# bacpop/ska.rust

Measured on AMD Instinct MI355X. Metric: genomes/sec ska build+align, 1 000x5 Mbp k=31; bit-exact vs CPU, higher is better.
Workload: dtype u64

## Files before the change

ska.rust_amd/csrc/skx_api.cpp:

```cpp
#include "skx_internal.h"
#include "../../include/skx_host.h"
#include <algorithm>
#include <atomic>
#include <chrono>
#include <cmath>
#include <cstdarg>
#include <cstddef>
#include <cstdio>
#include <cstring>
#include <map>
#include <memory>
#include <mutex>
#include <numeric>
#include <optional>
#include <unordered_map>
#include <thread>
#include <cerrno>
#include <fcntl.h>
#include <sys/mman.h>
#include <sys/stat.h>
#include <unistd.h>

using namespace skx;

// ... 1057 lines not shown
    int missing = 0;
    SKX_HIP(hipMemcpyAsync(&missing, d_flag.p, 4, hipMemcpyDeviceToHost, st));
    SKX_HIP(hipStreamSynchronize(st));
    SKX_HIP(hipGetLastError());
    if (missing) { set_error("row keyset does not contain every split k-mer of the samples"); return SKX_EINVAL; }
    *out = a.release();
    return SKX_OK;
    });
}

static PiecesRowsArgs pieces_args(skx_array *a)
{
    PiecesRowsArgs pa{};
    const skx_pieces *pc = a->pieces; const skx_keyset *rows = a->lazy_rows;
    pa.pieces = pc->data.p; pa.plen = pc->plen.p; pa.perm = pc->perm.p; pa.nrank = pc->nrank.p; pa.cap = pc->cap; pa.n_samples = (int)a->names.size();
    pa.ncnt = rows->ncnt.p; pa.roff = rows->roff.p;
    return pa;
}
static void launch_assemble_lazy(skx_array *a, const AssembleArgs &aa, hipStream_t st, int mode, uint32_t n_blocks = 0)
{
    if (a->lazy_rows->wide) launch_assemble_wide(aa, st, mode, n_blocks); else launch_assemble(aa, st, mode, n_blocks);
}
static AssembleArgs lazy_args(skx_array *a, int *d_flag)
{
    AssembleArgs aa{};
    skx_keyset *rows = a->lazy_rows;
    aa.d = a->lazy_dict->view(); aa.logN = rows->logN; aa.stage = rows->stage.p; aa.stride = rows->stride; aa.ncnt = rows->ncnt.p; aa.roff = rows->roff.p;
    aa.matrix = nullptr; aa.pitch = 0; aa.col_present = a->present.p; aa.col_unambig = a->unambig.p; aa.col_mask = a->mask.p;
    aa.max_rows = rows->max_rows; aa.missing = d_flag;
    return aa;
// ... 184 lines not shown
        if (logQ > bits || attempt > 3) return not_taken("row blocks kept overflowing (a sample that is one repeat, or far more rows than the probe saw)");
        const uint64_t nsub = 1ull << logQ;
        const double mean = u_est / (double)nsub;
        const uint32_t cap = ranks_for(mean), nslots = slots_for(cap);
        const uint64_t amp = 1ull << (logQ - logB);
        const uint64_t amp_max = region_cap > (wide ? LDS_SORT_MAX_WIDE : LDS_SORT_MAX) ? 32 : 8;
        if (amp > amp_max && (double)raw_sum * (double)amp > 4e8) return not_taken("too many row blocks per region: every region would be read too often");
        if (!pass_ok(logQ, nslots, cap)) return not_taken("no row-block split that fits the LDS");
        std::unique_ptr<skx_keyset> ks(new skx_keyset());
        ks->ctx = ctx; ks->k = d->k; ks->rc = d->rc; ks->logN = logQ; ks->hp = d->hp; ks->wh = d->wh; ks->wide = wide; ks->stride = cap;
        std::unique_ptr<skx_pieces> pc(new skx_pieces());
        pc->cap = cap; pc->logQ = logQ;
        SKX_TRY(ks->stage.alloc(nsub * cap * wpk)); SKX_TRY(ks->ncnt.alloc(nsub));
        if (pc->data.alloc(nsub * (uint64_t)S * (cap / 2)) != SKX_OK) return not_taken("no room for the pieces");
        SKX_TRY(pc->plen.alloc(nsub * (uint64_t)S + 2)); SKX_TRY(pc->perm.alloc(nsub * cap)); SKX_TRY(pc->nrank.alloc(nsub));
        SKX_TRY(d_flag.zero(st));
        aa.logQ = logQ; aa.nslots = nslots; aa.cap = cap;
        aa.rounds = 1; aa.bar = nullptr;
        DevBuf<int> d_bar;
        {
            int cus = 0; (void)hipDeviceGetAttribute(&cus, hipDeviceAttributeMultiprocessorCount, ctx->device);
            uint64_t g = nsub;
            while (g > (uint64_t)std::max(cus, 1) && g % 2 == 0) g /= 2;
            if (g <= (uint64_t)std::max(cus, 1) && nsub % g == 0 && g % (8 * amp) == 0 && logB >= 3) {
                aa.rounds = (uint32_t)(nsub / g);
                SKX_TRY(d_bar.alloc(2ull << logB)); SKX_TRY(d_bar.zero(st)); aa.bar = d_bar.p;
            }
        }
        aa.pieces = pc->data.p; aa.plen = pc->plen.p; aa.perm = pc->perm.p; aa.nrank = pc->nrank.p;
        aa.stage = ks->stage.p; aa.stride = cap; aa.ncnt = ks->ncnt.p;
        { KernelTimer kt(ctx, &ctx->tm.append); if (wide) launch_append_wide(aa, st); else launch_append(aa, region_cap, st); }
        int ov = 0;
        SKX_HIP(hipMemcpyAsync(&ov, d_flag.p, 4, hipMemcpyDeviceToHost, st));
        SKX_HIP(hipStreamSynchronize(st));
        SKX_HIP(hipGetLastError());
        if (getenv("SKX_DEBUG")) fprintf(stderr, "[skx] append%s: logQ=%d (x%llu per region) cap=%u slots=%u rows~%.0f -> %s\n", wide ? " (128-bit keys)" : "", logQ, (unsigned long long)amp, cap, nslots, u_est, ov ? "overflow" : "ok");
        if (ov & 4) return not_taken("the table's bytes are not at LDS address 0");
        if (ov) continue;
        SKX_TRY(keyset_finish(ks.get()));
        ctx->merge_path = wide ? "append128" : "append64";
        ks_out = std::move(ks); pc_out = std::move(pc);
        return SKX_OK;
    }
}
// ... 23 lines not shown
        SKX_HIP(hipMemcpyAsync(blk->roff.p, ks->roff.p, (nsub + 1) * 8, hipMemcpyDeviceToDevice, st));
        blk->total = U; blk->max_rows = ks->max_rows;
    }
    std::unique_ptr<skx_array> a(new skx_array());
    a->ctx = ctx; a->k = d->k; a->rc = d->rc; a->k_bits = d->key_bits; a->hp = d->hp; a->wh = d->wh; a->version = skx_version();
    for (int i = 0; i < S; i++) a->names.emplace_back(names && names[i] ? names[i] : "");
    a->n_rows = a->n_kmers = U; a->pitch = 0; a->engine_order = true; a->stats_ready = true;
    SKX_TRY(a->present.alloc(U)); SKX_TRY(a->unambig.alloc(U)); SKX_TRY(a->mask.alloc(U)); SKX_TRY(a->keys.alloc(U * (d->wide() ? 2 : 1))); SKX_TRY(a->vcount.alloc(U));
    if (U) {
        skx_keyset *src = g ? g : ks;
        if (src->wide) launch_gather_keys_wide((const u128 *)src->stage.p, src->stride, g ? g->ncnt.p : blk->ncnt.p, g ? g->roff.p : blk->roff.p, 1 << src->logN, (u128 *)a->keys.p, st);
        else launch_gather_keys(src->stage.p, src->stride, g ? g->ncnt.p : blk->ncnt.p, g ? g->roff.p : blk->roff.p, 1 << src->logN, a->keys.p, 0, src->hp, st);
        if (g) { SKX_TRY(a->present.zero(st)); SKX_TRY(a->unambig.zero(st)); SKX_TRY(a->mask.zero(st)); SKX_TRY(a->vcount.zero(st)); }
        StageTimer t(ctx, &ctx->tm.assemble);
        KernelTimer kt(ctx, &ctx->tm.pieces_stats);
        launch_pieces_stats(pc->data.p, pc->plen.p, pc->perm.p, pc->nrank.p, blk->ncnt.p, blk->roff.p, pc->cap, S, 1 << logQ, a->present.p, a->unambig.p, a->mask.p, a->vcount.p, st);
    }
    SKX_HIP(hipStreamSynchronize(st));
    SKX_HIP(hipGetLastError());
    a->pieces = pc.release(); a->lazy_rows = blk.release();
    *out = a.release();
    return SKX_OK;
}
static int merge_append(skx_ctx *ctx, skx_dictset *d, const char *const *names, skx_array **out)
{
    std::unique_ptr<skx_keyset> ks; std::unique_ptr<skx_pieces> pc;
    const int r = append_pass(ctx, d, ks, pc);
    if (r != SKX_OK) return r;
    return array_over_pieces(ctx, d, ks.get(), pc.release(), nullptr, names, out);
}

// ... 250 lines not shown
    if (counts) for (uint64_t i = 0; i < U; i++) counts[i] = pres[idx[i]];
    return SKX_OK;
    });
}

extern "C" int skx_array_sample_kmers(skx_array *a, int64_t *out)
{
    return skx_guarded([&]() -> int {
    skx_ctx *ctx = a->ctx; hipStream_t st = ctx->stream;
    SKX_HIP(hipSetDevice(ctx->device));
    const size_t S = a->names.size();
    if (a->pieces) {
        skx_pieces *pc = a->pieces;
        if (pc->sample_cells.size() != S) {
            DevBuf<unsigned long long> d; SKX_TRY(d.alloc(S)); SKX_TRY(d.zero(st));
            launch_pieces_cells(pc->data.p, pc->plen.p, pc->cap, (int)S, 1 << pc->logQ, d.p, st);
            std::vector<unsigned long long> h(S);
            SKX_HIP(hipMemcpyAsync(h.data(), d.p, S * 8, hipMemcpyDeviceToHost, st));
            SKX_HIP(hipStreamSynchronize(st));
            pc->sample_cells.assign(h.begin(), h.end());
        }
        for (size_t i = 0; i < S; i++) out[i] = (int64_t)pc->sample_cells[i];
        return SKX_OK;
    }
    if (a->lazy()) { for (size_t i = 0; i < S; i++) out[i] = (int64_t)a->lazy_dict->sample_size[i]; return SKX_OK; }
    DevBuf<unsigned long long> d; SKX_TRY(d.alloc(S)); SKX_TRY(d.zero(st));
    launch_row_nonmissing(a->matrix.p, a->pitch, (int)S, a->n_rows, d.p, st);
    std::vector<unsigned long long> h(S);
    SKX_HIP(hipMemcpyAsync(h.data(), d.p, S * 8, hipMemcpyDeviceToHost, st));
    SKX_HIP(hipStreamSynchronize(st));
    for (size_t i = 0; i < S; i++) out[i] = (int64_t)h[i];
// ... 1 lines not shown
    });
}

extern "C" int skx_array_pieces_info(skx_array *a, uint64_t *piece_bytes, uint64_t *row_blocks, uint32_t *ranks_per_block)
{
    return skx_guarded([&]() -> int {
    if (!a) { set_error("bad arguments"); return SKX_EINVAL; }
    if (piece_bytes) *piece_bytes = 0;
    if (row_blocks) *row_blocks = 0;
    if (ranks_per_block) *ranks_per_block = 0;
    const skx_pieces *pc = a->pieces;
    if (!pc) return SKX_OK;
    skx_ctx *ctx = a->ctx; hipStream_t st = ctx->stream;
    SKX_HIP(hipSetDevice(ctx->device));
    const uint64_t n = ((uint64_t)1 << pc->logQ) * a->names.size();
    std::vector<uint16_t> h(n);
    SKX_HIP(hipMemcpyAsync(h.data(), pc->plen.p, n * 2, hipMemcpyDeviceToHost, st));
    SKX_HIP(hipStreamSynchronize(st));
    uint64_t b = 0;
    for (uint16_t v : h) b += ((uint64_t)v + 31) / 32 * 16;
    if (piece_bytes) *piece_bytes = b;
    if (row_blocks) *row_blocks = (uint64_t)1 << pc->logQ;
    if (ranks_per_block) *ranks_per_block = pc->cap;
    return SKX_OK;
    });
}

static int array_compact(skx_array *a, DevBuf<uint8_t> &keep, DevBuf<uint64_t> &pos, uint64_t kept, int mask_ambig, bool vcount_from_unambig,
                         bool keys_follow)
{
    skx_ctx *ctx = a->ctx; hipStream_t st = ctx->stream;
    const uint64_t U = a->n_rows; const size_t S = a->names.size();
    const bool filter_ambig_as_missing = vcount_from_unambig;
    if (kept == U && !mask_ambig) {
        if (filter_ambig_as_missing && U) SKX_HIP(hipMemcpyAsync(a->vcount.p, a->unambig.p, U * 4, hipMemcpyDeviceToDevice, st));
// ... 990 lines not shown
```

ska.rust_amd/csrc/skx_append.hip:

```cpp
#include "skx_device.h"
#include <cstdlib>
#include <type_traits>

namespace skx {

typedef uint32_t u32x4 __attribute__((ext_vector_type(4)));
typedef const u32x4 __attribute__((address_space(1))) *g4_t;

#ifdef SKX_AP_PROF
__device__ unsigned long long g_ap_prof[16];
#define AP_PROF_START unsigned long long tprof = __builtin_readcyclecounter(), tacc[12] = {0, 0, 0, 0, 0, 0, 0, 0, 0, 0, 0, 0}
#define AP_PROF(i) do { const unsigned long long t_ = __builtin_readcyclecounter(); tacc[(i)] += t_ - tprof; tprof = t_; } while (0)
#define AP_PROF_FLUSH() do { for (int i_ = 0; i_ < 12; i_++) if (tacc[i_] && (i_ >= 6 || (threadIdx.x & 63) == 0)) atomicAdd(&g_ap_prof[i_], tacc[i_]); } while (0)
extern "C" void skx_debug_phase_prof(unsigned long long *out, int reset)
{
    unsigned long long h[16];
    (void)hipDeviceSynchronize();
    (void)hipMemcpyFromSymbol(h, HIP_SYMBOL(g_ap_prof), sizeof(h));
    for (int i = 0; i < 16; i++) out[i] = h[i];
    if (reset) { for (auto &x : h) x = 0; (void)hipMemcpyToSymbol(HIP_SYMBOL(g_ap_prof), h, sizeof(h)); }
}
#else
#define AP_PROF_START do { } while (0)
#define AP_PROF(i) do { } while (0)
// ... 347 lines not shown
#endif
                }
#endif
            }
            if (last_chunk) {
                while (qw != qbase) { batch(std::false_type{}); AP_PROF(2); while (nsq >= 64u) { slow_batch(); AP_PROF(3); } }
                while (nsq) { slow_batch(); AP_PROF(3); }
            }
            AP_PROF(1);
            if (last_chunk) {
                if (!COUNT_ONLY) {
                    uint32_t n = *lds_vol(&s_ctl[CTL_NROWS]);
                    n = __builtin_amdgcn_readfirstlane(n);
                    if (n > cap) n = cap;
                    uint8_t *dst = piece0 + (uint64_t)s * (cap / 2);
                    for (uint32_t v = lane; v * 32u < n; v += 64u) {
                        uint4 *src = reinterpret_cast<uint4 *>(rb) + v;
                        const uint4 x = *src;
                        *reinterpret_cast<uint4 *>(dst + v * 16u) = x;
                        *src = make_uint4(0u, 0u, 0u, 0u);
                    }
                    if (lane == 0) a.plen[j * (uint64_t)S + s] = (uint16_t)n;
                }
                AP_PROF(4);
                if (!more) break;
                s += AP_WAVES; c = 0; off_c = off_n; cnt_c = cnt_n;
                if (AP_RESYNC > 0) {
                    const int it = (s - wv) / AP_WAVES;
                    if (xmap && A > 1u && a.bar && it % (AP_RESYNC > 0 ? AP_RESYNC : 1) == 0 && it <= (S - AP_WAVES) / AP_WAVES) {
                        __syncthreads();
                        if (tid == 0) {
                            int *ctr = a.bar + (1 << a.logB) + region;
                            const int want = (int)A * (it / (AP_RESYNC > 0 ? AP_RESYNC : 1));
                            atomicAdd(ctr, 1);
                            for (int spin = 0; spin < (1 << 16) && __hip_atomic_load(ctr, __ATOMIC_RELAXED, __HIP_MEMORY_SCOPE_AGENT) < want; spin++) __builtin_amdgcn_s_sleep(4);
// ... 62 lines not shown
    } else {
        (void)hipFuncSetAttribute((const void *)append_kernel<COUNT_ONLY, false>, hipFuncAttributeMaxDynamicSharedMemorySize, (int)lds);
        hipLaunchKernelGGL((append_kernel<COUNT_ONLY, false>), dim3(blocks), dim3(AP_THREADS), lds, st, a);
    }
}
bool append_ok(int bits, int logB, int logQ, uint32_t region_cap, uint32_t nslots, uint32_t cap)
{
    const int rem = bits - logQ;
    (void)region_cap;
    return logQ >= logB && rem >= 0 && rem <= 50 && cap % 128u == 0 && cap >= 128u && cap <= APPEND_MAX_CAP && nslots >= cap && (nslots & (nslots - 1u)) == 0u &&
           append_lds_bytes(nslots, cap, false) <= 160u * 1024u - 256u;
}
void launch_append(const AppendArgs &a, uint32_t region_cap, hipStream_t st) { (void)region_cap; launch_append_t<false>(a, (1u << a.logQ) / a.rounds, st); }
void launch_append_probe(const AppendArgs &a, uint32_t region_cap, unsigned blocks, hipStream_t st) { (void)region_cap; launch_append_t<true>(a, blocks, st); }

__global__ __launch_bounds__(256) void pieces_stats_kernel(const uint8_t *pieces, const uint16_t *plen, const uint16_t *perm, const uint32_t *nrank, const uint32_t *ncnt,
                                                           const uint64_t *roff, uint32_t cap, int S, uint32_t *o_present, uint32_t *o_unambig, uint32_t *o_mask,
                                                           uint32_t *o_vcount, int force_direct, uint32_t stage)
{
    constexpr int W = 4;
    extern __shared__ __attribute__((aligned(16))) uint16_t s_stage[];
    const uint32_t PS_STAGE = stage;
    uint16_t *const s_pr = s_stage, *const s_un = s_stage + stage, *const s_mk = s_stage + 2 * (size_t)stage;
    const uint64_t j = blockIdx.x;
    const uint32_t nr = nrank[j], nrows = ncnt[j];
    const uint64_t r0 = roff[j];
    const uint32_t d = blockIdx.y * 256u + threadIdx.x;
    if (blockIdx.y * 256u * 8u * W >= nr && !(blockIdx.y == 0 && nrows)) return;
    const bool staged = gridDim.y == 1 && nrows <= PS_STAGE && !force_direct;
    if (staged) {
        for (uint32_t p = threadIdx.x; p < nrows; p += 256) { s_pr[p] = 0; s_un[p] = 0; s_mk[p] = 0; }
        __syncthreads();
    }
    const int lane = threadIdx.x & 63, wv = threadIdx.x >> 6;
    const uint16_t *pl = plen + j * (uint64_t)S;
    const uint4 *col = reinterpret_cast<const uint4 *>(pieces + j * (uint64_t)S * (cap / 2)) + d;
    const uint32_t step = cap / 32;
    const bool mine = d * 32u < nr;
    uint32_t pN[W], aN[W];
    uint32_t pE[W], pO[W], aE[W], aO[W], uni[W];
    uint32_t PE0[W], PE1[W], PO0[W], PO1[W], AE0[W], AE1[W], AO0[W], AO1[W];
#pragma unroll
    for (int w = 0; w < W; w++) { pN[w] = aN[w] = 0; pE[w] = pO[w] = aE[w] = aO[w] = uni[w] = 0; PE0[w] = PE1[w] = PO0[w] = PO1[w] = AE0[w] = AE1[w] = AO0[w] = AO1[w] = 0; }
    auto nibfold = [&]() {
#pragma unroll
        for (int w = 0; w < W; w++) {
            pE[w] += pN[w] & 0x0F0F0F0Fu; pO[w] += (pN[w] >> 4) & 0x0F0F0F0Fu; aE[w] += aN[w] & 0x0F0F0F0Fu; aO[w] += (aN[w] >> 4) & 0x0F0F0F0Fu;
            pN[w] = aN[w] = 0;
        }
    };
// ... 5 lines not shown
            AE0[w] += aE[w] & 0x00FF00FFu; AE1[w] += (aE[w] >> 8) & 0x00FF00FFu; AO0[w] += aO[w] & 0x00FF00FFu; AO1[w] += (aO[w] >> 8) & 0x00FF00FFu;
            pE[w] = pO[w] = aE[w] = aO[w] = 0;
        }
    };
    auto take = [&](int w, uint32_t x) {
        uint32_t t = x | (x >> 1); t |= t >> 2;
        const uint32_t nz = t & 0x11111111u;
        const uint32_t y = x & (x - nz);
        uint32_t u = y | (y >> 1); u |= u >> 2;
        const uint32_t am = u & 0x11111111u;
        pN[w] += nz; aN[w] += am;
        uni[w] |= x;
    };
    for (int s0 = 0, since = 0, nib = 0; s0 < S; s0 += 64) {
        const uint32_t plv = s0 + lane < S ? (uint32_t)pl[s0 + lane] : 0u;
        const int n = S - s0 < 64 ? S - s0 : 64;
#pragma unroll 1
        for (int i0 = 0; i0 < n; i0 += 4) {
            if (nib == 12) { nibfold(); nib = 0; }
            nib += 4;
            uint4 x[4];
#pragma unroll
            for (int u = 0; u < 4; u++) {
                const uint32_t l = (uint32_t)__builtin_amdgcn_readlane((int)plv, (i0 + u) & 63);
                x[u] = make_uint4(0u, 0u, 0u, 0u);
                if (mine && i0 + u < n && d * 32u < l) x[u] = col[(uint64_t)(s0 + i0 + u) * step];
            }
#pragma unroll
            for (int u = 0; u < 4; u++) { take(0, x[u].x); take(1, x[u].y); take(2, x[u].z); take(3, x[u].w); }
        }
        since += 64;
        if (since >= 192) { fold(); since = 0; nib = 0; }
    }
    fold();
    const uint16_t *pj = perm + j * (uint64_t)cap;
    if (mine) {
#pragma unroll
        for (int w = 0; w < W; w++) {
            uint32_t pres[8], amb[8];
            pres[0] = PE0[w] & 0xFFFFu; pres[4] = PE0[w] >> 16; pres[2] = PE1[w] & 0xFFFFu; pres[6] = PE1[w] >> 16;
            pres[1] = PO0[w] & 0xFFFFu; pres[5] = PO0[w] >> 16; pres[3] = PO1[w] & 0xFFFFu; pres[7] = PO1[w] >> 16;
// ... 27 lines not shown
        uint32_t pp = 0xFFFFu; bool hit = false;
        if (rr < rk1) {
            pp = pj[rr];
            if (pp < nrows) {
                if (staged) hit = s_un[pp] != s_pr[pp];
                else hit = __hip_atomic_load(&o_unambig[r0 + pp], __ATOMIC_RELAXED, __HIP_MEMORY_SCOPE_AGENT) != __hip_atomic_load(&o_present[r0 + pp], __ATOMIC_RELAXED, __HIP_MEMORY_SCOPE_AGENT);
            }
        }
        unsigned long long todo = __ballot(hit);
        while (todo) {
            const int src = __builtin_ctzll(todo);
            todo &= todo - 1;
            const uint32_t r = rb + (uint32_t)src, prow = (uint32_t)__shfl((int)pp, src, 64);
            uint32_t m = 0;
            for (int t = lane; t < S; t += 64) {
                if ((uint32_t)pl[t] <= r) continue;
                const uint32_t x = *(reinterpret_cast<const uint32_t *>(pieces + (j * (uint64_t)S + t) * (cap / 2)) + (r >> 3));
                const uint32_t nib = (x >> ((r & 7u) * 4u)) & 15u;
                if (nib) m |= 1u << nib;
            }
#pragma unroll
            for (int dd = 32; dd >= 1; dd >>= 1) m |= __shfl_xor(m, dd, 64);
            if (lane == 0) { if (staged) s_mk[prow] = (uint16_t)m; else o_mask[r0 + prow] = m; }
        }
    }
    if (!staged) return;
    __syncthreads();
    for (uint32_t p = threadIdx.x; p < nrows; p += 256) {
        const uint32_t pr = s_pr[p];
        o_present[r0 + p] = pr; o_vcount[r0 + p] = pr;
        o_unambig[r0 + p] = s_un[p]; o_mask[r0 + p] = s_mk[p];
    }
}
void launch_pieces_stats(const uint8_t *pieces, const uint16_t *plen, const uint16_t *perm, const uint32_t *nrank, const uint32_t *ncnt, const uint64_t *roff, uint32_t cap,
                         int n_samples, int n_blocks, uint32_t *present, uint32_t *unambig, uint32_t *mask, uint32_t *vcount, hipStream_t st)
{
    if (n_blocks <= 0) return;
    const unsigned gy = (cap / 32 + 255u) / 256u;
    static const int direct = knob("stats_direct") ? 1 : 0;
    const uint32_t stage = (cap + 63u) / 64u * 64u;
    hipLaunchKernelGGL(pieces_stats_kernel, dim3((unsigned)n_blocks, gy), dim3(256), (size_t)stage * 6, st, pieces, plen, perm, nrank, ncnt, roff, cap, n_samples, present, unambig, mask, vcount,
                       direct, stage);
}
__global__ __launch_bounds__(256) void pieces_cells_kernel(const uint8_t *pieces, const uint16_t *plen, uint32_t cap, int S, unsigned long long *out)
{
    const uint64_t j = blockIdx.x;
    const int lane = threadIdx.x & 63;
    for (int s = blockIdx.y * 4 + (threadIdx.x >> 6); s < S; s += gridDim.y * 4) {
        const uint32_t pl = plen[j * (uint64_t)S + s];
        const uint32_t *src = reinterpret_cast<const uint32_t *>(pieces + (j * (uint64_t)S + s) * (cap / 2));
        uint32_t c = 0;
        for (uint32_t i = lane; i < (pl + 7u) / 8u; i += 64) { const uint32_t x = src[i]; uint32_t t = x | (x >> 1); t |= t >> 2; c += (uint32_t)__popc(t & 0x11111111u); }
#pragma unroll
        for (int dd = 32; dd >= 1; dd >>= 1) c += __shfl_xor(c, dd, 64);
        if (lane == 0 && c) atomicAdd(&out[s], (unsigned long long)c);
    }
}
void launch_pieces_cells(const uint8_t *pieces, const uint16_t *plen, uint32_t cap, int n_samples, int n_blocks, unsigned long long *out, hipStream_t st)
{
    if (n_blocks <= 0 || n_samples <= 0) return;
    unsigned gy = (unsigned)((n_samples + 3) / 4); if (gy > 16) gy = 16;
    hipLaunchKernelGGL(pieces_cells_kernel, dim3((unsigned)n_blocks, gy), dim3(256), 0, st, pieces, plen, cap, n_samples, out);
}
__global__ __launch_bounds__(256) void region_totals_kernel(const uint32_t *raw, int logB, unsigned long long *out)
{
    __shared__ unsigned long long s_sum[256];
    const uint64_t B = 1ull << logB;
    unsigned long long t = 0;
    for (uint64_t b = threadIdx.x; b < B; b += 256) t += raw[(uint64_t)blockIdx.x * B + b];
    s_sum[threadIdx.x] = t;
    __syncthreads();
    for (int d = 128; d >= 1; d >>= 1) { if ((int)threadIdx.x < d) s_sum[threadIdx.x] += s_sum[threadIdx.x + d]; __syncthreads(); }
    if (threadIdx.x == 0) out[blockIdx.x] = s_sum[0];
}
void launch_region_totals(const uint32_t *raw, int n_samples, int logB, unsigned long long *out, hipStream_t st)
{
    if (n_samples > 0) hipLaunchKernelGGL(region_totals_kernel, dim3((unsigned)n_samples), dim3(256), 0, st, raw, logB, out);
}

constexpr int PR_WAVES = 8;
__device__ static inline uint32_t ap_iupac4(uint32_t m)
{
    const uint32_t idx = m & 0x07070707u;
    const uint32_t lo = __builtin_amdgcn_perm(0x48595754u, 0x4D43412Du, idx);
    const uint32_t hi = __builtin_amdgcn_perm(0x4E42444Bu, 0x56535247u, idx);
    const uint32_t sel = ((m >> 3) & 0x01010101u) * 0xFFu;
    return (hi & sel) | (lo & ~sel);
}
template <bool KEPT>
__global__ __launch_bounds__(64 * PR_WAVES) void pieces_rows_kernel(PiecesRowsArgs a)
{
    extern __shared__ __attribute__((aligned(16))) unsigned char s_raw[];
    const uint32_t cap = a.cap;
    uint16_t *s_src = reinterpret_cast<uint16_t *>(s_raw);
    uint32_t *s_piece = reinterpret_cast<uint32_t *>(s_raw + (((size_t)cap + 16) * 2 + 15) / 16 * 16);
    const uint64_t j = (uint64_t)blockIdx.x + a.j_base;
    const uint32_t n = a.ncnt[j];
    if (n == 0) return;
    const uint64_t r0 = a.roff[j];
    const uint64_t k0 = KEPT ? a.kpos[r0] : 0;
    const uint32_t nout = KEPT ? (uint32_t)(a.kpos[r0 + n] - k0) : n;
    if (nout == 0) return;
    const int tid = threadIdx.x, lane = tid & 63, wv = tid >> 6;
    const uint64_t ocol = KEPT ? k0 : r0 - a.col_base;
    const uint32_t shift = (uint32_t)(ocol & 3u);
    const uint32_t ndw = (nout + shift + 3u) / 4u;
    const uint16_t *pj = a.perm + j * (uint64_t)cap;
    const uint32_t nr = a.nrank[j];
    const int S = a.n_samples;
    const int s_lo = blockIdx.y * a.samples_per_wg, s_hi = s_lo + a.samples_per_wg < S ? s_lo + a.samples_per_wg : S;
    uint32_t *pc = s_piece + (size_t)wv * (cap / 8 + 4);
    const unsigned char *pcb = reinterpret_cast<const unsigned char *>(pc);
    const uint32_t nrw = (nr + 7u) / 8u;
    if (lane < 4) pc[cap / 8 + lane] = 0u;
    for (uint32_t t0 = 0; t0 < nout + shift; t0 += cap) {
        for (uint32_t i = tid; i < cap + 16u; i += blockDim.x) s_src[i] = (uint16_t)cap;
        __syncthreads();
        for (uint32_t r = tid; r < nr; r += blockDim.x) {
            const uint32_t p = pj[r];
            if (p == 0xFFFFu || p >= n) continue;
            uint32_t sc;
            if (!KEPT) sc = shift + p;
            else if (a.keep[r0 + p] == 1) sc = shift + (uint32_t)(a.kpos[r0 + p] - k0);
            else continue;
            if (sc >= t0 && sc < t0 + cap) s_src[sc - t0] = (uint16_t)r;
        }
        __syncthreads();
        const uint32_t v_lo = t0 / 4u, v_hi = (t0 + cap) / 4u < ndw ? (t0 + cap) / 4u : ndw;
        for (int s = s_lo + wv; s < s_hi; s += PR_WAVES) {
            const uint32_t pl = a.plen[j * (uint64_t)S + s];
            const uint32_t plw = (pl + 7u) / 8u;
            const uint32_t *src = reinterpret_cast<const uint32_t *>(a.pieces + (j * (uint64_t)S + s) * (cap / 2));
            {
                const uint4 *src4 = reinterpret_cast<const uint4 *>(src);
                uint4 *pc4 = reinterpret_cast<uint4 *>(pc);
                for (uint32_t i = lane; i < (nrw + 3u) / 4u; i += 64) {
                    uint4 x = 4u * i < plw ? src4[i] : make_uint4(0u, 0u, 0u, 0u);
                    if (4u * i + 1u >= plw) x.y = 0u;
                    if (4u * i + 2u >= plw) x.z = 0u;
                    if (4u * i + 3u >= plw) x.w = 0u;
                    pc4[i] = x;
                }
            }
            __builtin_amdgcn_wave_barrier();
            unsigned char *dst = a.out + (uint64_t)s * a.pitch + (ocol - shift);
            for (uint32_t v = v_lo + lane; v < v_hi; v += 64) {
                const uint2 rr = *reinterpret_cast<const uint2 *>(s_src + 4u * (v - v_lo));
                const uint32_t ra = rr.x & 0xFFFFu, rb = rr.x >> 16, rc = rr.y & 0xFFFFu, rd = rr.y >> 16;
                const uint32_t na = ((uint32_t)pcb[ra >> 1] >> ((ra & 1u) * 4u)) & 15u, nb = ((uint32_t)pcb[rb >> 1] >> ((rb & 1u) * 4u)) & 15u;
                const uint32_t nc = ((uint32_t)pcb[rc >> 1] >> ((rc & 1u) * 4u)) & 15u, nd = ((uint32_t)pcb[rd >> 1] >> ((rd & 1u) * 4u)) & 15u;
                uint32_t m = na | (nb << 8) | (nc << 16) | (nd << 24);
                uint32_t word = ap_iupac4(m);
// ... 39 lines not shown
```

ska.rust_amd/csrc/skx_append_wide.inc:

```
namespace skx {

constexpr uint32_t AW_Q = 192, AW_SQ = 64;
constexpr int AW_CH = 8;
typedef volatile unsigned long long __attribute__((address_space(3))) *lds_vol64_t;
__device__ static inline lds_vol64_t lds_vol64(void *p) { return (lds_vol64_t)(__attribute__((address_space(3))) void *)p; }

static inline size_t append_wide_lds_bytes(uint32_t nslots, uint32_t cap, bool count_only)
{
    size_t b = (size_t)(nslots + AP_PAD) * 17 + (size_t)AP_WAVES * (AW_Q + AW_SQ) * 16 + CTL_WORDS * 4;
    if (!count_only) b += (size_t)AP_WAVES * (cap / 8) * 4;
    return b;
}

template <bool COUNT_ONLY, int QS, int PD>
__global__ __launch_bounds__(AP_THREADS) void append_wide_kernel(AppendArgs a)
{
    extern __shared__ __attribute__((aligned(16))) unsigned char s_raw[];
    const uint32_t total_slots = a.nslots + AP_PAD;
    const uint32_t cap = a.cap, rbw = cap / 8;
    unsigned char *s_fp = s_raw;
    unsigned long long *s_tab = reinterpret_cast<unsigned long long *>(s_raw + total_slots);
    u32x4 *s_q = reinterpret_cast<u32x4 *>(s_tab + 2 * (size_t)total_slots);
    uint32_t *s_ctl = reinterpret_cast<uint32_t *>(s_q + (size_t)AP_WAVES * (AW_Q + AW_SQ));
    uint32_t *s_rb = s_ctl + CTL_WORDS;
// ... 211 lines not shown
                case 0: AW_FILTER_STEP(0); break; case 1: AW_FILTER_STEP(64); break; case 2: AW_FILTER_STEP(128); break; case 3: AW_FILTER_STEP(192); break;
                case 4: AW_FILTER_STEP(256); break; case 5: AW_FILTER_STEP(320); break; case 6: AW_FILTER_STEP(384); break; default: AW_FILTER_STEP(448); break;
                }
#undef AW_FILTER_STEP
                issue_one(r, nb1);
                while (qw >= qfull) batch(std::true_type{});
            }
            if (last_chunk) {
                while (qw != qbase) batch(std::false_type{});
                while (nsq) slow_batch();
                if (!COUNT_ONLY) {
                    uint32_t n = *lds_vol(&s_ctl[CTL_NROWS]);
                    n = __builtin_amdgcn_readfirstlane(n);
                    if (n > cap) n = cap;
                    uint8_t *dst = piece0 + (uint64_t)s * (cap / 2);
                    for (uint32_t v = lane; v * 32u < n; v += 64u) {
                        uint4 *src = reinterpret_cast<uint4 *>(rb) + v;
                        const uint4 x = *src;
                        *reinterpret_cast<uint4 *>(dst + v * 16u) = x;
                        *src = make_uint4(0u, 0u, 0u, 0u);
                    }
                    if (lane == 0) a.plen[j * (uint64_t)S + s] = (uint16_t)n;
                }
                if (!more) break;
                s += AP_WAVES; c = 0; off_c = off_n; cnt_c = cnt_n;
                if (AP_RESYNC > 0) {
                    const int it = (s - wv) / AP_WAVES;
                    if (xmap && A > 1u && a.bar && it % (AP_RESYNC > 0 ? AP_RESYNC : 1) == 0 && it <= (S - AP_WAVES) / AP_WAVES) {
                        __syncthreads();
                        if (tid == 0) {
                            int *ctr = a.bar + (1 << a.logB) + region;
                            const int want = (int)A * (it / (AP_RESYNC > 0 ? AP_RESYNC : 1));
                            atomicAdd(ctr, 1);
                            for (int spin = 0; spin < (1 << 16) && __hip_atomic_load(ctr, __ATOMIC_RELAXED, __HIP_MEMORY_SCOPE_AGENT) < want; spin++) __builtin_amdgcn_s_sleep(4);
                        }
// ... 79 lines not shown
```

ska.rust_amd/csrc/skx_device.h:

```cpp
#pragma once
#include <hip/hip_runtime.h>
#include <stdint.h>

namespace skx {

long knob(const char *name, long absent = 0);
int extract_tile_bases(int logB);
constexpr int MAX_LOGB = 13;
constexpr uint64_t EMPTY64 = ~0ull;

struct HashParams {
    int bits;
    int hb;
    uint32_t hmask;
    uint32_t c[4];
};
HashParams make_hash_params(int k);
__host__ __device__ inline uint32_t hround(uint32_t v, uint32_t c, int hb) { return (v * c) >> (32 - hb); }
__host__ __device__ inline void hmix_halves(uint32_t &L, uint32_t &R, const HashParams &p)
{
    L ^= hround(R, p.c[0], p.hb); R ^= hround(L, p.c[1], p.hb);
}
__host__ __device__ inline uint64_t hmix(uint64_t x, const HashParams &p)
{
// ... 92 lines not shown
    uint64_t col_base = 0;
    const uint8_t *keep = nullptr; const uint64_t *kpos = nullptr;
    int mask_ambig = 0;
};
void launch_assemble(const AssembleArgs &a, hipStream_t st, int mode = 0, uint32_t n_blocks = 0);
bool union_side_ok(const DictView &d, int logN, uint32_t stride);
void launch_union_side(const DictView &d, int logN, uint64_t *stage, uint32_t stride, uint32_t *ncnt, uint32_t table_slots, int *overflow,
                       uint16_t *side, uint16_t *perm, hipStream_t st);
void launch_assemble_side(const AssembleArgs &a, const uint16_t *side, const uint16_t *perm, hipStream_t st, bool wide = false);
void launch_compose_perm(const uint64_t *l_stage, uint32_t l_stride, const uint32_t *l_ncnt, const uint16_t *l_perm, int l_logN, const uint64_t *g_stage,
                         uint32_t g_stride, const uint32_t *g_ncnt, const uint64_t *g_roff, int g_logN, int bits, uint16_t *g_perm, uint32_t *g_n,
                         uint64_t *g_base, uint32_t *g_max, int *bad, hipStream_t st);
void launch_union_side_wide(const DictView &d, int logN, u128 *stage, uint32_t stride, uint32_t *ncnt, uint32_t table_slots, int *overflow,
                            uint16_t *side, uint16_t *perm, hipStream_t st);

constexpr uint32_t APPEND_MAX_CAP = 6016, APPEND_MAX_SLOTS = 8192;
struct AppendArgs {
    const uint64_t *words; const uint64_t *off; const uint32_t *raw;
    int n_samples, logB, bits, logQ;
    uint32_t nslots, cap;
    uint8_t *pieces; uint16_t *plen; uint16_t *perm; uint32_t *nrank;
    uint64_t *stage; uint32_t stride; uint32_t *ncnt;
    unsigned long long *probe;
    int *overflow;
    uint32_t rounds = 1;
    int *bar = nullptr;
};
bool append_ok(int bits, int logB, int logQ, uint32_t region_cap, uint32_t nslots, uint32_t cap);
void launch_append(const AppendArgs &a, uint32_t region_cap, hipStream_t st);
void launch_append_probe(const AppendArgs &a, uint32_t region_cap, unsigned blocks, hipStream_t st);
constexpr uint32_t APPEND_WIDE_MAX_CAP = 3072, APPEND_WIDE_MAX_SLOTS = 4096;
bool append_wide_ok(int bits, int logB, int logQ, uint32_t nslots, uint32_t cap);
void launch_append_wide(const AppendArgs &a, hipStream_t st);
void launch_append_wide_probe(const AppendArgs &a, unsigned blocks, hipStream_t st);
void launch_pieces_stats(const uint8_t *pieces, const uint16_t *plen, const uint16_t *perm, const uint32_t *nrank, const uint32_t *ncnt, const uint64_t *roff, uint32_t cap,
                         int n_samples, int n_blocks, uint32_t *present, uint32_t *unambig, uint32_t *mask, uint32_t *vcount, hipStream_t st);
void launch_pieces_cells(const uint8_t *pieces, const uint16_t *plen, uint32_t cap, int n_samples, int n_blocks, unsigned long long *out, hipStream_t st);
void launch_region_totals(const uint32_t *raw, int n_samples, int logB, unsigned long long *out, hipStream_t st);
struct PiecesRowsArgs {
    const uint8_t *pieces; const uint16_t *plen; const uint16_t *perm; const uint32_t *nrank; uint32_t cap; int n_samples;
    const uint32_t *ncnt; const uint64_t *roff;
    uint8_t *out; uint64_t pitch;
    uint32_t j_base = 0; uint64_t col_base = 0;
    const uint8_t *keep = nullptr; const uint64_t *kpos = nullptr;
    int mask_ambig = 0;
    int samples_per_wg = 0;
};
void launch_pieces_rows(const PiecesRowsArgs &a, uint32_t n_blocks, hipStream_t st);

void launch_gather_keys(const uint64_t *stage, uint32_t stride, const uint32_t *ncnt, const uint64_t *roff, int n_sub,
                        uint64_t *out, int unhash, HashParams hp, hipStream_t st);
void launch_hash_keys(const uint64_t *keys, uint64_t *words, uint64_t n, HashParams hp, hipStream_t st);
void launch_keys_cbor(const uint64_t *words, uint64_t n, HashParams hp, uint8_t *out, int *short_key, hipStream_t st);
void launch_unhash_dict(const uint64_t *words, uint64_t n, uint64_t *keys, uint8_t *bases, HashParams hp, hipStream_t st);

// ... 118 lines not shown
```

ska.rust_amd/csrc/skx_internal.h:

```cpp
#pragma once
#include "../../include/skx.h"
#include "skx_device.h"
#include <atomic>
#include <chrono>
#include <cstdio>
#include <condition_variable>
#include <functional>
#include <memory>
#include <mutex>
#include <new>
#include <thread>
#include <sys/types.h>
#include <stdexcept>
#include <string>
#include <vector>

namespace skx {

void set_error(const char *fmt, ...);

int hip_fail(hipError_t e, const char *what);

#define SKX_HIP(call) do { hipError_t e_ = (call); if (e_ != hipSuccess) return skx::hip_fail(e_, #call); } while (0)
#define SKX_TRY(call) do { int r_ = (call); if (r_ != SKX_OK) return r_; } while (0)
// ... 68 lines not shown
    skx::DevBuf<uint64_t> off;
    skx::DevBuf<uint32_t> raw;
    skx::DevBuf<uint32_t> ucnt;
    skx::DevBuf<uint16_t> sidx;
    int sb = 0;
    std::vector<uint64_t> sample_size;
    bool sorted = true;
    uint32_t region_cap = 0; uint64_t maxlen = 0;
    std::vector<uint64_t> raw_total;
    skx::DictView view() const { return skx::DictView{words.p, off.p, ucnt.p, n, logB, wide() ? wh.bits : hp.bits, sidx.p, sb}; }
};

struct skx_pieces {
    skx::DevBuf<uint8_t> data;
    skx::DevBuf<uint16_t> plen;
    skx::DevBuf<uint16_t> perm;
    skx::DevBuf<uint32_t> nrank;
    uint32_t cap = 0; int logQ = 0;
    std::vector<uint64_t> sample_cells;
};

struct skx_keyset {
    skx_ctx *ctx = nullptr;
    int k = 0, rc = 0, logN = 0;
    skx::HashParams hp{};
    skx::WideHash wh{};
    bool wide = false;
    int wpk() const { return wide ? 2 : 1; }
    uint32_t stride = 0, max_rows = 0;
    uint64_t total = 0;
// ... 222 lines not shown
```

Before: 29000.

## Track nonzero 16-byte piece groups with ballot bitmasks and skip zero groups

The append kernels now write only nonzero 16-byte groups of each sample's piece and record a per-group occupancy bitmask built with a wave ballot. The stats, cells and rows kernels read this mask and load only occupied groups, and the rows kernel also bounds its loop by the highest referenced rank. This cuts global memory reads and writes for sparse pieces, at the cost of an extra mask buffer and mask loads. A debug knob can poison the piece buffer to check that unwritten groups are never read.

```diff
diff --git a/ska.rust_amd/csrc/skx_api.cpp b/ska.rust_amd/csrc/skx_api.cpp
--- a/ska.rust_amd/csrc/skx_api.cpp
+++ b/ska.rust_amd/csrc/skx_api.cpp
@@ -1095,6 +1095,7 @@
     PiecesRowsArgs pa{};
     const skx_pieces *pc = a->pieces; const skx_keyset *rows = a->lazy_rows;
     pa.pieces = pc->data.p; pa.plen = pc->plen.p; pa.perm = pc->perm.p; pa.nrank = pc->nrank.p; pa.cap = pc->cap; pa.n_samples = (int)a->names.size();
+    pa.gmask = pc->gmask.p;
     pa.ncnt = rows->ncnt.p; pa.roff = rows->roff.p;
     return pa;
 }
@@ -1309,6 +1310,8 @@
         SKX_TRY(ks->stage.alloc(nsub * cap * wpk)); SKX_TRY(ks->ncnt.alloc(nsub));
         if (pc->data.alloc(nsub * (uint64_t)S * (cap / 2)) != SKX_OK) return not_taken("no room for the pieces");
         SKX_TRY(pc->plen.alloc(nsub * (uint64_t)S + 2)); SKX_TRY(pc->perm.alloc(nsub * cap)); SKX_TRY(pc->nrank.alloc(nsub));
+        SKX_TRY(pc->gmask.alloc(nsub * (uint64_t)S * piece_mask_words(cap)));
+        if (knob("piece_poison")) SKX_HIP(hipMemsetAsync(pc->data.p, 0xFF, nsub * (uint64_t)S * (cap / 2), st));
         SKX_TRY(d_flag.zero(st));
         aa.logQ = logQ; aa.nslots = nslots; aa.cap = cap;
         aa.rounds = 1; aa.bar = nullptr;
@@ -1322,7 +1325,7 @@
                 SKX_TRY(d_bar.alloc(2ull << logB)); SKX_TRY(d_bar.zero(st)); aa.bar = d_bar.p;
             }
         }
-        aa.pieces = pc->data.p; aa.plen = pc->plen.p; aa.perm = pc->perm.p; aa.nrank = pc->nrank.p;
+        aa.pieces = pc->data.p; aa.plen = pc->plen.p; aa.perm = pc->perm.p; aa.nrank = pc->nrank.p; aa.gmask = pc->gmask.p;
         aa.stage = ks->stage.p; aa.stride = cap; aa.ncnt = ks->ncnt.p;
         { KernelTimer kt(ctx, &ctx->tm.append); if (wide) launch_append_wide(aa, st); else launch_append(aa, region_cap, st); }
         int ov = 0;
@@ -1376,7 +1379,7 @@
         if (g) { SKX_TRY(a->present.zero(st)); SKX_TRY(a->unambig.zero(st)); SKX_TRY(a->mask.zero(st)); SKX_TRY(a->vcount.zero(st)); }
         StageTimer t(ctx, &ctx->tm.assemble);
         KernelTimer kt(ctx, &ctx->tm.pieces_stats);
-        launch_pieces_stats(pc->data.p, pc->plen.p, pc->perm.p, pc->nrank.p, blk->ncnt.p, blk->roff.p, pc->cap, S, 1 << logQ, a->present.p, a->unambig.p, a->mask.p, a->vcount.p, st);
+        launch_pieces_stats(pc->data.p, pc->plen.p, pc->gmask.p, pc->perm.p, pc->nrank.p, blk->ncnt.p, blk->roff.p, pc->cap, S, 1 << logQ, a->present.p, a->unambig.p, a->mask.p, a->vcount.p, st);
     }
     SKX_HIP(hipStreamSynchronize(st));
     SKX_HIP(hipGetLastError());
@@ -1657,7 +1660,7 @@
         skx_pieces *pc = a->pieces;
         if (pc->sample_cells.size() != S) {
             DevBuf<unsigned long long> d; SKX_TRY(d.alloc(S)); SKX_TRY(d.zero(st));
-            launch_pieces_cells(pc->data.p, pc->plen.p, pc->cap, (int)S, 1 << pc->logQ, d.p, st);
+            launch_pieces_cells(pc->data.p, pc->plen.p, pc->gmask.p, pc->cap, (int)S, 1 << pc->logQ, d.p, st);
             std::vector<unsigned long long> h(S);
             SKX_HIP(hipMemcpyAsync(h.data(), d.p, S * 8, hipMemcpyDeviceToHost, st));
             SKX_HIP(hipStreamSynchronize(st));
@@ -1689,11 +1692,15 @@
     skx_ctx *ctx = a->ctx; hipStream_t st = ctx->stream;
     SKX_HIP(hipSetDevice(ctx->device));
     const uint64_t n = ((uint64_t)1 << pc->logQ) * a->names.size();
+    const uint32_t mw = piece_mask_words(pc->cap);
     std::vector<uint16_t> h(n);
+    std::vector<unsigned long long> hm(n * mw);
     SKX_HIP(hipMemcpyAsync(h.data(), pc->plen.p, n * 2, hipMemcpyDeviceToHost, st));
+    SKX_HIP(hipMemcpyAsync(hm.data(), pc->gmask.p, n * mw * 8, hipMemcpyDeviceToHost, st));
     SKX_HIP(hipStreamSynchronize(st));
     uint64_t b = 0;
-    for (uint16_t v : h) b += ((uint64_t)v + 31) / 32 * 16;
+    for (uint64_t i = 0; i < n; i++)
+        for (uint32_t w = 0; w * 2048u < h[i]; w++) b += (uint64_t)__builtin_popcountll(hm[i * mw + w]) * 16;
     if (piece_bytes) *piece_bytes = b;
     if (row_blocks) *row_blocks = (uint64_t)1 << pc->logQ;
     if (ranks_per_block) *ranks_per_block = pc->cap;
diff --git a/ska.rust_amd/csrc/skx_append.hip b/ska.rust_amd/csrc/skx_append.hip
--- a/ska.rust_amd/csrc/skx_append.hip
+++ b/ska.rust_amd/csrc/skx_append.hip
@@ -385,11 +385,18 @@
                     n = __builtin_amdgcn_readfirstlane(n);
                     if (n > cap) n = cap;
                     uint8_t *dst = piece0 + (uint64_t)s * (cap / 2);
-                    for (uint32_t v = lane; v * 32u < n; v += 64u) {
-                        uint4 *src = reinterpret_cast<uint4 *>(rb) + v;
-                        const uint4 x = *src;
-                        *reinterpret_cast<uint4 *>(dst + v * 16u) = x;
-                        *src = make_uint4(0u, 0u, 0u, 0u);
+                    unsigned long long *gm = a.gmask + (j * (uint64_t)S + s) * piece_mask_words(cap);
+                    for (uint32_t v0 = 0; v0 * 32u < n; v0 += 64u) {
+                        const uint32_t v = v0 + (uint32_t)lane;
+                        bool nz = false;
+                        if (v * 32u < n) {
+                            uint4 *src = reinterpret_cast<uint4 *>(rb) + v;
+                            const uint4 x = *src;
+                            nz = (x.x | x.y | x.z | x.w) != 0u;
+                            if (nz) { *reinterpret_cast<uint4 *>(dst + v * 16u) = x; *src = make_uint4(0u, 0u, 0u, 0u); }
+                        }
+                        const unsigned long long word = __ballot(nz);
+                        if (lane == 0) gm[v0 >> 6] = word;
                     }
                     if (lane == 0) a.plen[j * (uint64_t)S + s] = (uint16_t)n;
                 }
@@ -482,7 +489,7 @@
 void launch_append(const AppendArgs &a, uint32_t region_cap, hipStream_t st) { (void)region_cap; launch_append_t<false>(a, (1u << a.logQ) / a.rounds, st); }
 void launch_append_probe(const AppendArgs &a, uint32_t region_cap, unsigned blocks, hipStream_t st) { (void)region_cap; launch_append_t<true>(a, blocks, st); }
 
-__global__ __launch_bounds__(256) void pieces_stats_kernel(const uint8_t *pieces, const uint16_t *plen, const uint16_t *perm, const uint32_t *nrank, const uint32_t *ncnt,
+__global__ __launch_bounds__(256) void pieces_stats_kernel(const uint8_t *pieces, const uint16_t *plen, const unsigned long long *gmask, const uint16_t *perm, const uint32_t *nrank, const uint32_t *ncnt,
                                                            const uint64_t *roff, uint32_t cap, int S, uint32_t *o_present, uint32_t *o_unambig, uint32_t *o_mask,
                                                            uint32_t *o_vcount, int force_direct, uint32_t stage)
 {
@@ -502,6 +509,8 @@
     }
     const int lane = threadIdx.x & 63, wv = threadIdx.x >> 6;
     const uint16_t *pl = plen + j * (uint64_t)S;
+    const uint32_t mw = piece_mask_words(cap), wd = blockIdx.y * 4u + (uint32_t)wv;
+    const unsigned long long *gm = gmask + j * (uint64_t)S * mw;
     const uint4 *col = reinterpret_cast<const uint4 *>(pieces + j * (uint64_t)S * (cap / 2)) + d;
     const uint32_t step = cap / 32;
     const bool mine = d * 32u < nr;
@@ -537,6 +546,8 @@
     };
     for (int s0 = 0, since = 0, nib = 0; s0 < S; s0 += 64) {
         const uint32_t plv = s0 + lane < S ? (uint32_t)pl[s0 + lane] : 0u;
+        const unsigned long long gv = wd * 2048u < plv ? gm[(uint64_t)(s0 + lane) * mw + wd] : 0ull;
+        const uint32_t glo = (uint32_t)gv, ghi = (uint32_t)(gv >> 32);
         const int n = S - s0 < 64 ? S - s0 : 64;
 #pragma unroll 1
         for (int i0 = 0; i0 < n; i0 += 4) {
@@ -545,9 +556,9 @@
             uint4 x[4];
 #pragma unroll
             for (int u = 0; u < 4; u++) {
-                const uint32_t l = (uint32_t)__builtin_amdgcn_readlane((int)plv, (i0 + u) & 63);
+                const unsigned long long g = ((unsigned long long)(uint32_t)__builtin_amdgcn_readlane((int)ghi, (i0 + u) & 63) << 32) | (uint32_t)__builtin_amdgcn_readlane((int)glo, (i0 + u) & 63);
                 x[u] = make_uint4(0u, 0u, 0u, 0u);
-                if (mine && i0 + u < n && d * 32u < l) x[u] = col[(uint64_t)(s0 + i0 + u) * step];
+                if (mine && i0 + u < n && ((g >> lane) & 1ull)) x[u] = col[(uint64_t)(s0 + i0 + u) * step];
             }
 #pragma unroll
             for (int u = 0; u < 4; u++) { take(0, x[u].x); take(1, x[u].y); take(2, x[u].z); take(3, x[u].w); }
@@ -605,7 +616,7 @@
             const uint32_t r = rb + (uint32_t)src, prow = (uint32_t)__shfl((int)pp, src, 64);
             uint32_t m = 0;
             for (int t = lane; t < S; t += 64) {
-                if ((uint32_t)pl[t] <= r) continue;
+                if ((uint32_t)pl[t] <= r || !((gm[(uint64_t)t * mw + (r >> 11)] >> ((r >> 5) & 63u)) & 1ull)) continue;
                 const uint32_t x = *(reinterpret_cast<const uint32_t *>(pieces + (j * (uint64_t)S + t) * (cap / 2)) + (r >> 3));
                 const uint32_t nib = (x >> ((r & 7u) * 4u)) & 15u;
                 if (nib) m |= 1u << nib;
@@ -623,35 +634,42 @@
         o_unambig[r0 + p] = s_un[p]; o_mask[r0 + p] = s_mk[p];
     }
 }
-void launch_pieces_stats(const uint8_t *pieces, const uint16_t *plen, const uint16_t *perm, const uint32_t *nrank, const uint32_t *ncnt, const uint64_t *roff, uint32_t cap,
+void launch_pieces_stats(const uint8_t *pieces, const uint16_t *plen, const unsigned long long *gmask, const uint16_t *perm, const uint32_t *nrank, const uint32_t *ncnt, const uint64_t *roff, uint32_t cap,
                          int n_samples, int n_blocks, uint32_t *present, uint32_t *unambig, uint32_t *mask, uint32_t *vcount, hipStream_t st)
 {
     if (n_blocks <= 0) return;
     const unsigned gy = (cap / 32 + 255u) / 256u;
-    static const int direct = knob("stats_direct") ? 1 : 0;
+    const int direct = knob("stats_direct") ? 1 : 0;
     const uint32_t stage = (cap + 63u) / 64u * 64u;
-    hipLaunchKernelGGL(pieces_stats_kernel, dim3((unsigned)n_blocks, gy), dim3(256), (size_t)stage * 6, st, pieces, plen, perm, nrank, ncnt, roff, cap, n_samples, present, unambig, mask, vcount,
+    hipLaunchKernelGGL(pieces_stats_kernel, dim3((unsigned)n_blocks, gy), dim3(256), (size_t)stage * 6, st, pieces, plen, gmask, perm, nrank, ncnt, roff, cap, n_samples, present, unambig, mask, vcount,
                        direct, stage);
 }
-__global__ __launch_bounds__(256) void pieces_cells_kernel(const uint8_t *pieces, const uint16_t *plen, uint32_t cap, int S, unsigned long long *out)
+__global__ __launch_bounds__(256) void pieces_cells_kernel(const uint8_t *pieces, const uint16_t *plen, const unsigned long long *gmask, uint32_t cap, int S, unsigned long long *out)
 {
     const uint64_t j = blockIdx.x;
     const int lane = threadIdx.x & 63;
     for (int s = blockIdx.y * 4 + (threadIdx.x >> 6); s < S; s += gridDim.y * 4) {
         const uint32_t pl = plen[j * (uint64_t)S + s];
-        const uint32_t *src = reinterpret_cast<const uint32_t *>(pieces + (j * (uint64_t)S + s) * (cap / 2));
+        const uint4 *src = reinterpret_cast<const uint4 *>(pieces + (j * (uint64_t)S + s) * (cap / 2));
+        const unsigned long long *gm = gmask + (j * (uint64_t)S + s) * piece_mask_words(cap);
         uint32_t c = 0;
-        for (uint32_t i = lane; i < (pl + 7u) / 8u; i += 64) { const uint32_t x = src[i]; uint32_t t = x | (x >> 1); t |= t >> 2; c += (uint32_t)__popc(t & 0x11111111u); }
+        for (uint32_t g0 = 0; g0 * 32u < pl; g0 += 64) {
+            if (!((gm[g0 >> 6] >> lane) & 1ull)) continue;
+            const uint4 x4 = src[g0 + lane];
+            const uint32_t xs[4] = {x4.x, x4.y, x4.z, x4.w};
+#pragma unroll
+            for (int w = 0; w < 4; w++) { const uint32_t x = xs[w]; uint32_t t = x | (x >> 1); t |= t >> 2; c += (uint32_t)__popc(t & 0x11111111u); }
+        }
 #pragma unroll
         for (int dd = 32; dd >= 1; dd >>= 1) c += __shfl_xor(c, dd, 64);
         if (lane == 0 && c) atomicAdd(&out[s], (unsigned long long)c);
     }
 }
-void launch_pieces_cells(const uint8_t *pieces, const uint16_t *plen, uint32_t cap, int n_samples, int n_blocks, unsigned long long *out, hipStream_t st)
+void launch_pieces_cells(const uint8_t *pieces, const uint16_t *plen, const unsigned long long *gmask, uint32_t cap, int n_samples, int n_blocks, unsigned long long *out, hipStream_t st)
 {
     if (n_blocks <= 0 || n_samples <= 0) return;
     unsigned gy = (unsigned)((n_samples + 3) / 4); if (gy > 16) gy = 16;
-    hipLaunchKernelGGL(pieces_cells_kernel, dim3((unsigned)n_blocks, gy), dim3(256), 0, st, pieces, plen, cap, n_samples, out);
+    hipLaunchKernelGGL(pieces_cells_kernel, dim3((unsigned)n_blocks, gy), dim3(256), 0, st, pieces, plen, gmask, cap, n_samples, out);
 }
 __global__ __launch_bounds__(256) void region_totals_kernel(const uint32_t *raw, int logB, unsigned long long *out)
 {
@@ -682,6 +700,7 @@
 __global__ __launch_bounds__(64 * PR_WAVES) void pieces_rows_kernel(PiecesRowsArgs a)
 {
     extern __shared__ __attribute__((aligned(16))) unsigned char s_raw[];
+    __shared__ uint32_t s_top;
     const uint32_t cap = a.cap;
     uint16_t *s_src = reinterpret_cast<uint16_t *>(s_raw);
     uint32_t *s_piece = reinterpret_cast<uint32_t *>(s_raw + (((size_t)cap + 16) * 2 + 15) / 16 * 16);
@@ -692,7 +711,7 @@
     const uint64_t k0 = KEPT ? a.kpos[r0] : 0;
     const uint32_t nout = KEPT ? (uint32_t)(a.kpos[r0 + n] - k0) : n;
     if (nout == 0) return;
-    const int tid = threadIdx.x, lane = tid & 63, wv = tid >> 6;
+    const int tid = threadIdx.x, lane = tid & 63, wv = __builtin_amdgcn_readfirstlane(tid >> 6);
     const uint64_t ocol = KEPT ? k0 : r0 - a.col_base;
     const uint32_t shift = (uint32_t)(ocol & 3u);
     const uint32_t ndw = (nout + shift + 3u) / 4u;
@@ -702,11 +721,14 @@
     const int s_lo = blockIdx.y * a.samples_per_wg, s_hi = s_lo + a.samples_per_wg < S ? s_lo + a.samples_per_wg : S;
     uint32_t *pc = s_piece + (size_t)wv * (cap / 8 + 4);
     const unsigned char *pcb = reinterpret_cast<const unsigned char *>(pc);
-    const uint32_t nrw = (nr + 7u) / 8u;
+    const uint32_t mw = piece_mask_words(cap);
+    typedef const unsigned long long __attribute__((address_space(4))) *cmask_t;
     if (lane < 4) pc[cap / 8 + lane] = 0u;
     for (uint32_t t0 = 0; t0 < nout + shift; t0 += cap) {
         for (uint32_t i = tid; i < cap + 16u; i += blockDim.x) s_src[i] = (uint16_t)cap;
+        if (tid == 0) s_top = 0u;
         __syncthreads();
+        uint32_t top = 0;
         for (uint32_t r = tid; r < nr; r += blockDim.x) {
             const uint32_t p = pj[r];
             if (p == 0xFFFFu || p >= n) continue;
@@ -714,9 +736,11 @@
             if (!KEPT) sc = shift + p;
             else if (a.keep[r0 + p] == 1) sc = shift + (uint32_t)(a.kpos[r0 + p] - k0);
             else continue;
-            if (sc >= t0 && sc < t0 + cap) s_src[sc - t0] = (uint16_t)r;
-        }
+            if (sc >= t0 && sc < t0 + cap) { s_src[sc - t0] = (uint16_t)r; top = r + 1u; }
+        }
+        if (top) atomicMax(&s_top, top);
         __syncthreads();
+        const uint32_t ngr = (s_top + 31u) / 32u;
         const uint32_t v_lo = t0 / 4u, v_hi = (t0 + cap) / 4u < ndw ? (t0 + cap) / 4u : ndw;
         for (int s = s_lo + wv; s < s_hi; s += PR_WAVES) {
             const uint32_t pl = a.plen[j * (uint64_t)S + s];
@@ -725,8 +749,12 @@
             {
                 const uint4 *src4 = reinterpret_cast<const uint4 *>(src);
                 uint4 *pc4 = reinterpret_cast<uint4 *>(pc);
-                for (uint32_t i = lane; i < (nrw + 3u) / 4u; i += 64) {
-                    uint4 x = 4u * i < plw ? src4[i] : make_uint4(0u, 0u, 0u, 0u);
+                const cmask_t gm = (cmask_t)(uintptr_t)(a.gmask + (j * (uint64_t)S + s) * mw);
+                for (uint32_t i0 = 0; i0 < ngr; i0 += 64) {
+                    const unsigned long long g = i0 * 32u < pl ? gm[i0 >> 6] : 0ull;
+                    const uint32_t i = i0 + (uint32_t)lane;
+                    if (i >= ngr) break;
+                    uint4 x = (g >> lane) & 1ull ? src4[i] : make_uint4(0u, 0u, 0u, 0u);
                     if (4u * i + 1u >= plw) x.y = 0u;
                     if (4u * i + 2u >= plw) x.z = 0u;
                     if (4u * i + 3u >= plw) x.w = 0u;
diff --git a/ska.rust_amd/csrc/skx_append_wide.inc b/ska.rust_amd/csrc/skx_append_wide.inc
--- a/ska.rust_amd/csrc/skx_append_wide.inc
+++ b/ska.rust_amd/csrc/skx_append_wide.inc
@@ -249,11 +249,18 @@
                     n = __builtin_amdgcn_readfirstlane(n);
                     if (n > cap) n = cap;
                     uint8_t *dst = piece0 + (uint64_t)s * (cap / 2);
-                    for (uint32_t v = lane; v * 32u < n; v += 64u) {
-                        uint4 *src = reinterpret_cast<uint4 *>(rb) + v;
-                        const uint4 x = *src;
-                        *reinterpret_cast<uint4 *>(dst + v * 16u) = x;
-                        *src = make_uint4(0u, 0u, 0u, 0u);
+                    unsigned long long *gm = a.gmask + (j * (uint64_t)S + s) * piece_mask_words(cap);
+                    for (uint32_t v0 = 0; v0 * 32u < n; v0 += 64u) {
+                        const uint32_t v = v0 + (uint32_t)lane;
+                        bool nz = false;
+                        if (v * 32u < n) {
+                            uint4 *src = reinterpret_cast<uint4 *>(rb) + v;
+                            const uint4 x = *src;
+                            nz = (x.x | x.y | x.z | x.w) != 0u;
+                            if (nz) { *reinterpret_cast<uint4 *>(dst + v * 16u) = x; *src = make_uint4(0u, 0u, 0u, 0u); }
+                        }
+                        const unsigned long long word = __ballot(nz);
+                        if (lane == 0) gm[v0 >> 6] = word;
                     }
                     if (lane == 0) a.plen[j * (uint64_t)S + s] = (uint16_t)n;
                 }
diff --git a/ska.rust_amd/csrc/skx_device.h b/ska.rust_amd/csrc/skx_device.h
--- a/ska.rust_amd/csrc/skx_device.h
+++ b/ska.rust_amd/csrc/skx_device.h
@@ -130,12 +130,14 @@
 void launch_union_side_wide(const DictView &d, int logN, u128 *stage, uint32_t stride, uint32_t *ncnt, uint32_t table_slots, int *overflow,
                             uint16_t *side, uint16_t *perm, hipStream_t st);
 
+constexpr uint32_t piece_mask_words(uint32_t cap) { return (cap / 32u + 63u) / 64u; }
 constexpr uint32_t APPEND_MAX_CAP = 6016, APPEND_MAX_SLOTS = 8192;
 struct AppendArgs {
     const uint64_t *words; const uint64_t *off; const uint32_t *raw;
     int n_samples, logB, bits, logQ;
     uint32_t nslots, cap;
     uint8_t *pieces; uint16_t *plen; uint16_t *perm; uint32_t *nrank;
+    unsigned long long *gmask;
     uint64_t *stage; uint32_t stride; uint32_t *ncnt;
     unsigned long long *probe;
     int *overflow;
@@ -149,12 +151,13 @@
 bool append_wide_ok(int bits, int logB, int logQ, uint32_t nslots, uint32_t cap);
 void launch_append_wide(const AppendArgs &a, hipStream_t st);
 void launch_append_wide_probe(const AppendArgs &a, unsigned blocks, hipStream_t st);
-void launch_pieces_stats(const uint8_t *pieces, const uint16_t *plen, const uint16_t *perm, const uint32_t *nrank, const uint32_t *ncnt, const uint64_t *roff, uint32_t cap,
+void launch_pieces_stats(const uint8_t *pieces, const uint16_t *plen, const unsigned long long *gmask, const uint16_t *perm, const uint32_t *nrank, const uint32_t *ncnt, const uint64_t *roff, uint32_t cap,
                          int n_samples, int n_blocks, uint32_t *present, uint32_t *unambig, uint32_t *mask, uint32_t *vcount, hipStream_t st);
-void launch_pieces_cells(const uint8_t *pieces, const uint16_t *plen, uint32_t cap, int n_samples, int n_blocks, unsigned long long *out, hipStream_t st);
+void launch_pieces_cells(const uint8_t *pieces, const uint16_t *plen, const unsigned long long *gmask, uint32_t cap, int n_samples, int n_blocks, unsigned long long *out, hipStream_t st);
 void launch_region_totals(const uint32_t *raw, int n_samples, int logB, unsigned long long *out, hipStream_t st);
 struct PiecesRowsArgs {
     const uint8_t *pieces; const uint16_t *plen; const uint16_t *perm; const uint32_t *nrank; uint32_t cap; int n_samples;
+    const unsigned long long *gmask;
     const uint32_t *ncnt; const uint64_t *roff;
     uint8_t *out; uint64_t pitch;
     uint32_t j_base = 0; uint64_t col_base = 0;
diff --git a/ska.rust_amd/csrc/skx_internal.h b/ska.rust_amd/csrc/skx_internal.h
--- a/ska.rust_amd/csrc/skx_internal.h
+++ b/ska.rust_amd/csrc/skx_internal.h
@@ -106,6 +106,7 @@
 struct skx_pieces {
     skx::DevBuf<uint8_t> data;
     skx::DevBuf<uint16_t> plen;
+    skx::DevBuf<unsigned long long> gmask;
     skx::DevBuf<uint16_t> perm;
     skx::DevBuf<uint32_t> nrank;
     uint32_t cap = 0; int logQ = 0;
```

Result: no change. 28990 (-0.0%).
